# Wallacoloo/libfriendship

Hardware: AMD Instinct MI355X
Metric: Msamples/sec at 4096 partials x 64 voices; achieved HBM GB/s vs roofline (higher is better)
Workload: dtype f32

## Files before the change

libfriendship_amd/csrc/engine.cpp:

```cpp
#include <hip/hip_runtime_api.h>

#include <algorithm>
#include <cfloat>
#include <cmath>
#include <cstdio>
#include <cstdlib>
#include <chrono>
#include <cstring>
#include <map>
#include <sstream>
#include <string>
#include <vector>

#include "../../include/friendship_render_ext.h"
#include "bankplan.hpp"
#include "callplan.hpp"
#include "comm.hpp"
#include "graph.hpp"
#include "jit.hpp"
#include "kernels.hpp"
#include "match.hpp"
#include "stage.hpp"
#include "streamplan.hpp"
#include "streamrows.hpp"
// ... 204 lines not shown
__attribute__((weak)) hipError_t launch_bank_stream_loops(const StreamBanksArgs &, const BankArgs &, const StreamProgArgs &, uint32_t, uint32_t, uint32_t, uint32_t, BankStreamInCtl *,
                                                          BankStreamInDev *, uint32_t, hipStream_t) {
    return hipErrorNotSupported;
}
__attribute__((weak)) hipError_t launch_track_window(const TrackWindowArgs &a, hipStream_t) {
    for (uint32_t r = 0; r < a.n_rows; ++r)
        for (uint64_t i = 0; i < a.back + a.n; ++i)
            a.dst[r][i] = i < a.back ? (a.tail[r] ? a.tail[r][(a.idx - a.back + i) & a.mask] : 0.0f) : (a.call[r] ? a.call[r][i - a.back] : 0.0f);
    return hipSuccess;
}

}

using namespace fr;

struct fr_renderer {
    int device = 0;
    int mode = FR_MODE_AUTO;
    int semantics = FR_SEMANTICS_REFERENCE;
    uint64_t history_frames = 0;
    hipStream_t stream = nullptr;
    Mirror mirror;
    std::vector<InSlot> slots;
    uint64_t n_vecs = 0;
    struct Seg { uint64_t first, last, len; };
    std::vector<Seg> segs;
    uint64_t head = 0;
    Plan plan;
    DevBuf d_out, d_in_table, d_stack_node, d_stack_time, d_stack_val, d_bank_ws, d_tickets;
    PinnedBuf h_in_stage, h_out_stage;
    uint32_t track_from = 0xFFFFFFFFu;
    uint32_t dense_total_rows = 0;
    const float *call_tracks = nullptr;
    uint64_t call_track_stride = 0, call_track_rows = 0;
    DevBuf d_tracks_stage;
    uint64_t track_history = 0, tail_cap = 0;
    DevBuf d_tail, d_track_win;
    uint32_t tail_rows = 0;
    uint64_t tail_end = 0;
    uint64_t tail_launches = 0;
    std::vector<std::pair<uint32_t, DevInput>> track_dev;
    bool tail_on() const { return track_history != 0 && track_from != 0xFFFFFFFFu; }
    DevBuf d_chunk_ws, d_chunk_rows;
    uint32_t d_chunk_rows_n = 0;
    uint32_t stage_block_env = 0;
    bool host_out_mapped = false, host_rows_mapped = true;
    size_t host_small_bytes = 96u << 10;
    bool host_direct = true;
    bool host_stream = true;
    PinnedBuf h_row_flags;
    DevBuf d_row_done;
    uint32_t host_seq = 0;
    std::vector<uint32_t> stream_pending;
    struct FlagOut { uint32_t *host_flags = nullptr; uint32_t *row_done = nullptr; uint32_t value = 0; } flag_out;
    bool can_stream_rows(uint32_t n_slots, uint64_t n_times) const {
        if (!host_stream || sharded() || !plan_current(n_slots) || plan.banks.empty()) return false;
        if (!plan.sp.progs.empty() || plan.sp.uses_rings() || !plan.pull_rows.empty() || !plan.sp.split.empty()) return false;
        size_t voices = 0;
        for (const BankStage &bs : plan.banks) {
            if (!plan_bank_launch(bs, n_times, true).publishes_rows) return false;
            voices += bs.grp.rows.size();
        }
        return voices == n_slots;
    }
    std::vector<std::pair<char *, size_t>> registered;
    bool host_trace = false;
    double trace_us[3] = {0, 0, 0};
    uint64_t trace_n = 0;
    hipEvent_t ev_last = nullptr;
    hipStream_t last_stream = nullptr;
    bool last_pending = false;
    bool last_independent = false;
    bool used_scratch = false;
    bool host_pipelines = false;
    bool overlapped_streams = false;
    bool plan_is_stateless(uint32_t n_slots) const {
        return plan_current(n_slots) && !plan.sp.uses_rings() && plan.sp.progs.empty() && plan.pull_rows.empty() && plan.sp.split.empty() &&
               !tail_on();
    }
    void order_after_previous(hipStream_t st, bool this_independent = false) {
        if (!last_pending) return;
        if (overlapped_streams && !this_independent) {
            HIP_CHECK(hipDeviceSynchronize());
            overlapped_streams = false;
            last_pending = false;
            return;
        }
        if (last_stream == st) return;
        if (last_independent && this_independent) {
            overlapped_streams = true;
            return;
        }
        if (!ev_last) HIP_CHECK(hipEventCreateWithFlags(&ev_last, hipEventDisableTiming));
        if (hipEventRecord(ev_last, last_stream) == hipSuccess) {
            HIP_CHECK(hipStreamWaitEvent(st, ev_last, 0));
        } else {
            (void)hipGetLastError();
            HIP_CHECK(hipDeviceSynchronize());
        }
        last_pending = false;
    }
    void remember_async(hipStream_t st, bool independent) {
        last_independent = independent;
        last_stream = st;
        last_pending = true;
    }
    ShardSpec shard;
    uint32_t shard_flags = 0;
    uint64_t shard_epoch = 0;
    std::unique_ptr<Transport> rccl;
    fr_comm host_comm{};
    bool has_host_comm = false;
    DevBuf d_ws, d_xrecv;
    hipStream_t xstream = nullptr;
    std::vector<hipEvent_t> x_events;
    uint32_t x_max_tiles = 4, x_min_tile = 1024;
    bool x_tiles_explicit = false;
    uint64_t exchange_bytes = 0;
    uint64_t exchange_calls = 0, exchange_tiles = 0;
    PinnedBuf h_xsend, h_xrecv;
    bool sharded() const { return shard.world > 1 && shard.mode != FR_SHARD_NONE; }
// ... 408 lines not shown
            for (uint32_t r = 0; r < n; ++r) if (need[r] && bank_ring[r]) voice_ring[r] = 1;
            while (!work.empty()) {
                const StageProg &pg = sp.progs[work.back()];
                work.pop_back();
                for (uint32_t k = 0; k < pg.n_instr; ++k) {
                    const StageInstr &in = sp.instrs[pg.first_instr + k];
                    if (in.op != S_READ && in.op != S_READ_DYN) continue;
                    if (bank_ring[in.buf]) voice_ring[in.buf] = 1;
                    else if (stored_by[in.buf] >= 0 && !in_set[(size_t)stored_by[in.buf]]) { in_set[(size_t)stored_by[in.buf]] = 1; work.push_back((uint32_t)stored_by[in.buf]); }
                }
            }
            add_voices(voice_ring);
            for (uint32_t r = 0; r < n; ++r) if (voice_ring[r]) now[r].valid_from = 0;
            for (size_t l = 0; l + 1 < sp.fused_level_first.size(); ++l) {
                std::vector<std::pair<uint32_t, uint32_t>> runs;
                for (uint32_t i = f0 + sp.fused_level_first[l]; i < f0 + sp.fused_level_first[l + 1]; ++i) {
                    if (!in_set[i]) continue;
                    add_run(runs, i);
                    for (uint32_t r : sp.prog_rings[i]) now[r].valid_from = 0;
                }
                if (!runs.empty()) rp.levels.push_back(std::move(runs));
            }
        }
        ring_state.repair_from = rp.from;
        ring_table.rings = std::move(now);
        ring_table.shard_epoch = shard_epoch;
        return rp;
    }
    std::vector<hipEvent_t> event_pool;
    std::string last_error;
    std::string jit_error;
    std::string plan_json_cache;

    ~fr_renderer() {
        (void)hipSetDevice(device);
        end_stream();
        for (TimerClass *tc : {&t_bank, &t_pull, &t_stage})
            for (auto &pr : tc->pending) { (void)hipEventDestroy(pr.first); (void)hipEventDestroy(pr.second); }
        for (hipEvent_t e : event_pool) (void)hipEventDestroy(e);
        for (Retired &g : graveyard) (void)hipEventDestroy(g.ev);
        if (ev_last) (void)hipEventDestroy(ev_last);
        if (ev_ring_move) (void)hipEventDestroy(ev_ring_move);
        for (hipEvent_t e : x_events) (void)hipEventDestroy(e);
        if (xstream) (void)hipStreamDestroy(xstream);
        if (!registered.empty()) (void)hipStreamSynchronize(stream);
        for (auto &rg : registered) { if (hipHostUnregister(rg.first) != hipSuccess) (void)hipGetLastError(); }
        if (host_trace && stream_trace_n)
            std::fprintf(stderr, "fr_stream_block over %llu blocks: ring + wait %.1f us, copy out %.1f us\n", (unsigned long long)stream_trace_n,
                         stream_trace_us[0] / stream_trace_n, stream_trace_us[1] / stream_trace_n);
        if (host_trace && trace_n)
            std::fprintf(stderr, "fr_fill_buffer phases over %llu calls (mapped out %d, mapped in %d): issue %.1f us, %s %.1f us, %s %.1f us\n",
                         (unsigned long long)trace_n, (int)host_out_mapped, (int)host_rows_mapped, trace_us[0] / trace_n,
                         host_out_mapped ? "wait" : "D2H issue", trace_us[1] / trace_n, host_out_mapped ? "CPU copy" : "wait", trace_us[2] / trace_n);
        if (stream) (void)hipStreamDestroy(stream);
    }

    uint64_t implicit_len(uint64_t slot) const {
        for (const Seg &s : segs) if (slot >= s.first && slot < s.last) return s.len;
        return 0;
    }

    hipEvent_t get_event() {
        if (!event_pool.empty()) { hipEvent_t e = event_pool.back(); event_pool.pop_back(); return e; }
        hipEvent_t e;
        HIP_CHECK(hipEventCreate(&e));
        return e;
    }
    struct Scope {
        fr_renderer *r; TimerClass *tc; hipStream_t s; hipEvent_t a = nullptr, b = nullptr;
        Scope(fr_renderer *rr, TimerClass *t, hipStream_t st) : r(rr), tc(t), s(st) {
            if (r->timing) { a = r->get_event(); b = r->get_event(); HIP_CHECK(hipEventRecord(a, s)); }
        }
        void done() {
            if (a) { HIP_CHECK(hipEventRecord(b, s)); tc->pending.emplace_back(a, b); a = nullptr; }
        }
    };
    void resolve(TimerClass &tc) {
        for (auto &pr : tc.pending) {
            HIP_CHECK(hipEventSynchronize(pr.second));
            float ms = 0;
            HIP_CHECK(hipEventElapsedTime(&ms, pr.first, pr.second));
            tc.ms += ms;
            tc.launches += 1;
            event_pool.push_back(pr.first);
            event_pool.push_back(pr.second);
        }
        tc.pending.clear();
    }

    bool delay_observed = false;
    uint64_t delay_observed_max = 1u << 20;
    struct Hull {
        float lo = 0.0f, hi = 0.0f;
        uint32_t flags = 0;
        bool known = true;
    };
    std::vector<Hull> hulls;
    uint64_t lookback_growths = 0;
    uint64_t range_launches = 0;
    uint64_t deferred_len = 0;
    PinnedBuf h_range;
    static bool widen(Hull &h, float lo, float hi, uint32_t flags) {
        const bool w = lo < h.lo || hi > h.hi || (flags & ~h.flags) != 0;
        h.lo = std::min(h.lo, lo);
        h.hi = std::max(h.hi, hi);
        h.flags |= flags;
// ... 758 lines not shown
            j.rows = d_chunk_rows.as<uint32_t>();
            j.out_stride = pt.blen;
        }
        if (bs.grp.tracks && pt.trk) {
            j.tracks = pt.trk->p;
            j.track_stride = pt.trk->stride;
            j.track_limit = pt.trk->limit;
        } else if (bs.grp.tracks && call_tracks) {
            if (pt.b0 != c.idx || pt.blen != c.n_times) throw Error(FR_ERR_UNSUPPORTED, "internal: a voice that reads tracks rendered over another window than the call's");
            j.tracks = call_tracks;
            j.track_stride = call_track_stride;
            j.track_limit = (uint32_t)std::min<uint64_t>((uint64_t)track_from + call_track_rows, 0xFFFFFFFFull);
        }
        note_bank_launch(bp, bs, pt.nv, pt.blen, flag_out.host_flags != nullptr);
        Scope sc(this, &t_bank, c.st);
        HIP_CHECK(launch_jit_bank(*bs.jit, j, c.st));
        if (bp.pieces_log2) {
            ChunkCombineArgs cc{};
            cc.ws = d_chunk_ws.as<float>();
            cc.out = a.out;
            cc.rows = a.rows;
            cc.out_stride = a.out_stride;
            cc.n_times = pt.blen;
            cc.n_voices = a.n_voices;
            cc.log2_c = bp.pieces_log2;
            HIP_CHECK(launch_chunk_combine(cc, c.st));
        }
        sc.done();
    }

    void launch_general_bank(const Call &c, BankStage &bs, const BankPart &pt, BankArgs &a) {
        a.groups = bs.d_groups.as<uint32_t>();
        a.group_off = bs.d_group_off.as<uint32_t>();
        a.hist_dst = nullptr;
        note_bank_launch(pt.bp, bs, pt.nv, pt.blen, flag_out.host_flags != nullptr);
        Scope sc(this, &t_bank, c.st);
        HIP_CHECK(launch_gbank(a, c.st));
        sc.done();
    }

    void launch_template_bank(const Call &c, BankStage &bs, const BankPart &pt, BankArgs &a) {
        const BankPlan &bp = pt.bp;
        if (a.hist_dst && !bp.appends_rows) throw Error(FR_ERR_DEVICE, "internal: deferred history append on a short call");
        a.chunk_log2 = bp.chunk_log2;
        a.frames_per_lane = bp.frames_per_lane;
        a.waves_per_group = bp.waves_per_group;
        a.small_call = bp.small_call;
        a.leaf_variant = bank_tune.leaf_variant;
        if (flag_out.host_flags) {
            if (!bp.publishes_rows) throw Error(FR_ERR_DEVICE, "internal: a bank launch cannot publish row flags");
            a.host_flags = flag_out.host_flags;
            a.row_done = flag_out.row_done;
            a.flag_value = flag_out.value;
        }
        if (bp.ws_floats) {
            used_scratch = true;
            d_bank_ws.ensure(bp.ws_floats * sizeof(float));
            a.ws = d_bank_ws.as<float>();
            if (bp.ticket_words) a.tickets = ticket_counters(bp.ticket_words, c.st);
        }
        note_bank_launch(bp, bs, pt.nv, pt.blen, flag_out.host_flags != nullptr);
        Scope sc(this, &t_bank, c.st);
        HIP_CHECK(launch_bank(a, c.st));
        sc.done();
    }

    void launch_bank_window(const Call &c, BankStage &bs, uint64_t b0, uint64_t blen, int64_t tile_off) {
        if (!(bs.grp.tracks && tail_on() && tile_off < 0 && b0 < c.idx && b0 + blen == c.idx + c.n_times)) {
            launch_bank_part(c, bs, b0, blen, tile_off, nullptr);
            return;
        }
        for (uint64_t s0 = b0; s0 < c.idx;) {
            const uint64_t pos = s0 & (tail_cap - 1);
            const uint64_t len = std::min(c.idx - s0, tail_cap - pos);
            TrackSrc ts{nullptr, tail_cap, 0};
            if (tail_rows) {
                ts.p = reinterpret_cast<const float *>(reinterpret_cast<uintptr_t>(d_tail.as<float>() + pos) - (uintptr_t)track_from * tail_cap * sizeof(float));
                ts.limit = (uint32_t)std::min<uint64_t>((uint64_t)track_from + tail_rows, 0xFFFFFFFFull);
            }
            launch_bank_part(c, bs, s0, len, -1, &ts);
            s0 += len;
        }
        launch_bank_part(c, bs, c.idx, c.n_times, -1, nullptr);
    }

    std::vector<DevInput> stage_tab;
    void fill_stage_tab(hipStream_t st) {
        const StagedPlan &sp = plan.sp;
        stage_tab.resize(sp.input_slots.size());
        for (size_t i = 0; i < stage_tab.size(); ++i) stage_tab[i] = dev_input(sp.input_slots[i]);
        if (stage_tab.size() > STAGE_INLINE_INPUTS) {
            d_in_table_stage.ensure(stage_tab.size() * sizeof(DevInput));
            HIP_CHECK(hipMemcpyAsync(d_in_table_stage.p, stage_tab.data(), stage_tab.size() * sizeof(DevInput), hipMemcpyHostToDevice, st));
            HIP_CHECK(hipStreamSynchronize(st));
        }
    }
    struct StageLaunch { const char *form; uint64_t stride; };
    template <class Args>
    void fill_stage_args(Args &a, const Call &c, const StageLaunch &how, uint64_t s0, uint64_t slen, bool carry_only) const {
        a.rings = d_rings.as<float>();
        a.ring_mask = ring_cap ? ring_cap - 1 : 0;
        a.n_inputs = (uint32_t)stage_tab.size();
        a.out = c.dst;
        a.n_times = c.n_times;
        a.idx = c.idx;
        a.w0 = s0;
// ... 630 lines not shown
}
fr_status fr_on_add_edge(fr_renderer *r, const fr_edge *edge) {
    return guarded(r, [&] {
        if (!edge) throw Error(FR_ERR_INVALID_ARG, "null edge");
        r->mirror.add_edge(*edge);
    });
}
fr_status fr_on_del_edge(fr_renderer *r, const fr_edge *edge) {
    return guarded(r, [&] {
        if (!edge) throw Error(FR_ERR_INVALID_ARG, "null edge");
        r->mirror.del_edge(*edge);
    });
}
fr_status fr_on_add_nodes(fr_renderer *r, const uint32_t *handles, const fr_effect *const *effects, size_t n) {
    return guarded(r, [&] {
        if (n && (!handles || !effects)) throw Error(FR_ERR_INVALID_ARG, "null array");
        r->mirror.nodes.reserve(r->mirror.nodes.size() + n);
        for (size_t i = 0; i < n; ++i) r->mirror.add_node(handles[i], effects[i]);
    });
}
fr_status fr_on_add_edges(fr_renderer *r, const fr_edge *edges, size_t n) {
    return guarded(r, [&] {
        if (n && !edges) throw Error(FR_ERR_INVALID_ARG, "null array");
        for (size_t i = 0; i < n; ++i) r->mirror.add_edge(edges[i]);
    });
}

fr_status fr_fill_buffer(fr_renderer *r, float *out, uint32_t n_slots, uint64_t n_times, uint64_t idx,
                         const float *in_data, const uint64_t *in_row_offsets, uint32_t n_in_rows) {
    return guarded(r, [&] {
        check_fill_args(out, n_slots, n_times, in_data, in_row_offsets, n_in_rows);
        HIP_CHECK(hipSetDevice(r->device));
        hipStream_t st = r->stream;
        r->order_after_previous(st);
        r->ensure_plan(n_slots, st);
        const auto snap = r->snapshot_store(idx);
        try {
        r->store_inputs(n_slots, n_times, idx, in_data, in_row_offsets, n_in_rows, false, st);
        size_t bytes = (size_t)n_slots * n_times * sizeof(float);
        uint32_t row_lo, row_hi;
        r->my_rows(n_slots, row_lo, row_hi);
        const bool gather = r->sharded() && (r->shard_flags & FR_SHARD_GATHER);
        using clk = std::chrono::steady_clock;
        const auto t_a = clk::now();
        float *direct = nullptr;
        if (!gather && bytes && r->host_direct)
            for (const auto &rg : r->registered)
                if ((char *)out >= rg.first && (char *)out + bytes <= rg.first + rg.second) {
                    void *dp = nullptr;
                    if (hipHostGetDevicePointer(&dp, out, 0) == hipSuccess) direct = (float *)dp;
                    else (void)hipGetLastError();
                    break;
                }
        if (direct) {
            r->execute(direct, n_slots, n_times, idx, st);
            HIP_CHECK(hipStreamSynchronize(st));
        } else if (bytes >= (256u << 10) && r->can_stream_rows(n_slots, n_times)) {
            r->h_out_stage.ensure(bytes);
            if ((size_t)n_slots * sizeof(uint32_t) > r->h_row_flags.bytes) {
                r->h_row_flags.ensure((size_t)n_slots * 2 * sizeof(uint32_t));
                std::memset(r->h_row_flags.p, 0, r->h_row_flags.bytes);
                r->host_seq = 0;
            }
            r->clean_counters(st);
            if ((size_t)n_slots * sizeof(uint32_t) > r->d_row_done.bytes) {
                r->d_row_done.ensure((size_t)n_slots * 2 * sizeof(uint32_t));
                HIP_CHECK(hipMemsetAsync(r->d_row_done.p, 0, r->d_row_done.bytes, st));
            }
            if (++r->host_seq == 0) {
                std::memset(r->h_row_flags.p, 0, r->h_row_flags.bytes);
                r->host_seq = 1;
            }
            const uint32_t seq = r->host_seq;
            r->flag_out.host_flags = r->h_row_flags.as_dev<uint32_t>();
            r->flag_out.row_done = r->d_row_done.as<uint32_t>();
            r->flag_out.value = seq;
            struct Clear { fr_renderer *r; ~Clear() { r->flag_out = fr_renderer::FlagOut{}; } } clear{r};
            r->execute(r->h_out_stage.as_dev<float>(), n_slots, n_times, idx, st);
            const uint32_t *flags = r->h_row_flags.as<uint32_t>();
            const float *stage = r->h_out_stage.as<float>();
            r->stream_pending.resize(n_slots);
            for (uint32_t i = 0; i < n_slots; ++i) r->stream_pending[i] = i;
            size_t left = n_slots;
            uint64_t idle = 0;
            while (left) {
                bool progress = false;
                for (size_t i = 0; i < left;) {
                    const uint32_t row = r->stream_pending[i];
                    if (__atomic_load_n(flags + row, __ATOMIC_ACQUIRE) == seq) {
                        std::memcpy(out + (size_t)row * n_times, stage + (size_t)row * n_times, n_times * sizeof(float));
                        r->stream_pending[i] = r->stream_pending[--left];
                        progress = true;
                    } else {
                        ++i;
                    }
                }
                if (!progress && (++idle & 0xFFFFu) == 0 && hipStreamQuery(st) != hipErrorNotReady) {
                    HIP_CHECK(hipStreamSynchronize(st));
                    for (size_t i = 0; i < left; ++i)
                        if (__atomic_load_n(flags + r->stream_pending[i], __ATOMIC_ACQUIRE) != seq)
                            throw Error(FR_ERR_DEVICE, "internal: a rendered row was never published to the host");
                }
            }
            HIP_CHECK(hipStreamSynchronize(st));
        } else if ((r->host_out_mapped || bytes <= r->host_small_bytes) && !gather) {
            r->h_out_stage.ensure(bytes);
            r->execute(r->h_out_stage.as_dev<float>(), n_slots, n_times, idx, st);
            const auto t_b = clk::now();
            HIP_CHECK(hipStreamSynchronize(st));
            const auto t_c = clk::now();
            const size_t off = (size_t)row_lo * n_times, cnt = (size_t)(row_hi - row_lo) * n_times;
            if (cnt) std::memcpy(out + off, r->h_out_stage.as<float>() + off, cnt * sizeof(float));
            if (r->host_trace) {
                r->trace_us[0] += std::chrono::duration<double, std::micro>(t_b - t_a).count();
                r->trace_us[1] += std::chrono::duration<double, std::micro>(t_c - t_b).count();
                r->trace_us[2] += std::chrono::duration<double, std::micro>(clk::now() - t_c).count();
                ++r->trace_n;
            }
        } else {
            r->d_out.ensure(bytes);
            r->execute(r->d_out.as<float>(), n_slots, n_times, idx, st);
            if (gather) {
                r->gather_rows(r->d_out.as<float>(), n_slots, n_times, st);
                if (r->shard.rank == 0) { row_lo = 0; row_hi = n_slots; }
            }
            const size_t off = (size_t)row_lo * n_times, cnt = (size_t)(row_hi - row_lo) * n_times;
            const auto t_b = clk::now();
            if (cnt) HIP_CHECK(hipMemcpyAsync(out + off, r->d_out.as<float>() + off, cnt * sizeof(float), hipMemcpyDeviceToHost, st));
            const auto t_c = clk::now();
            HIP_CHECK(hipStreamSynchronize(st));
            if (r->host_trace) {
                r->trace_us[0] += std::chrono::duration<double, std::micro>(t_b - t_a).count();
                r->trace_us[1] += std::chrono::duration<double, std::micro>(t_c - t_b).count();
                r->trace_us[2] += std::chrono::duration<double, std::micro>(clk::now() - t_c).count();
                ++r->trace_n;
            }
        }
        } catch (...) {
            r->rollback_store(snap);
            throw;
        }
        r->last_pending = false;
        r->head = idx + n_times;
    });
}

fr_status fr_fill_buffer_device(fr_renderer *r, float *d_out, uint32_t n_slots, uint64_t n_times, uint64_t idx,
                                const float *d_in_data, const uint64_t *in_row_offsets, uint32_t n_in_rows,
                                void *stream) {
    return guarded(r, [&] {
        check_fill_args(d_out, n_slots, n_times, d_in_data, in_row_offsets, n_in_rows);
        HIP_CHECK(hipSetDevice(r->device));
        hipStream_t st = (hipStream_t)stream;
        bool independent = r->plan_is_stateless(n_slots) && idx == r->head;
        for (uint32_t i = 0; independent && i < n_in_rows; ++i) independent = in_row_offsets[i + 1] - in_row_offsets[i] == n_times;
        r->host_pipelines = independent && r->last_pending && r->last_stream != st;
        struct Reset { fr_renderer *r; ~Reset() { r->host_pipelines = false; } } reset{r};
// ... 442 lines not shown
```

libfriendship_amd/csrc/kernels.hip:

```cpp
#include <hip/hip_runtime.h>

#include <cstdlib>
#include <type_traits>

#include "kernels.hpp"

#pragma clang fp contract(off)

namespace fr {

#ifdef FR_DIAG_STAMPS
__device__ unsigned long long *g_diag = nullptr;
#define FR_DIAG_MARK(slot)                                                                                                 \
    do {                                                                                                                   \
        if (g_diag && (threadIdx.x & 63u) == 0u) {                                                                         \
            unsigned long long v_ = __builtin_amdgcn_s_memrealtime();                                                      \
            if ((slot) == 3) v_ = (unsigned long long)__builtin_amdgcn_s_getreg(0xF804) | ((unsigned long long)(__builtin_amdgcn_s_getreg(0xF814) & 15u) << 32); \
            g_diag[((size_t)blockIdx.x * 16u + (threadIdx.x >> 6)) * 8u + (slot)] = v_;                                    \
            if ((slot) != 3) g_diag[((size_t)blockIdx.x * 16u + (threadIdx.x >> 6)) * 8u + 4u + (slot)] = __builtin_amdgcn_s_memtime(); \
        }                                                                                                                  \
    } while (0)
#else
#define FR_DIAG_MARK(slot) do { } while (0)
#endif
// ... 221 lines not shown
        res[f] = r;
    }
}

__device__ __forceinline__ bool leaves_all_negzero(const float2 *params, uint32_t n, float t, uint32_t tid, uint32_t nthreads) {
    bool ok = true;
    for (uint32_t k = tid; k < n && ok; k += nthreads) {
        float2 p = params[k];
        ok = __float_as_uint(bank_leaf<false, true>(t, p.x, p.y)) == 0x80000000u;
    }
    return ok;
}

template <bool FAST>
__device__ __attribute__((noinline)) bool wave_leaves_all_negzero(const float *params, uint32_t ngroups, float t, unsigned long long lanes) {
    const_f32_ptr p = (const_f32_ptr)params;
    const bool wanted = (lanes >> (threadIdx.x & 63u)) & 1ull;
    uint32_t all_and = 0xFFFFFFFFu, all_or = 0u;
    ParamGroup pa, pb;
    load_group(pa, p, 0);
    auto fold = [&](const ParamGroup &pg) {
#pragma unroll
        for (int j = 0; j < 8; ++j) {
            uint32_t b = __float_as_uint(bank_leaf<FAST, true>(t, pg.w[j], pg.A[j]));
            all_and &= b;
            all_or |= b;
        }
    };
    for (uint32_t g = 0; g < ngroups; g += 2) {
        const bool has_b = g + 1 < ngroups;
        __builtin_amdgcn_s_waitcnt(0xC07F);
        if (has_b) load_group(pb, p, g + 1);
        fold(pa);
        if (has_b) {
            __builtin_amdgcn_s_waitcnt(0xC07F);
            if (g + 2 < ngroups) load_group(pa, p, g + 2);
            fold(pb);
        }
        if (__ballot(wanted && all_and == 0x80000000u && all_or == 0x80000000u) == 0ull) {
            __builtin_amdgcn_s_waitcnt(0xC07F);
            return false;
        }
    }
    return all_and == 0x80000000u && all_or == 0x80000000u;
}

__device__ __forceinline__ float bank_time(const BankArgs &a, uint64_t ti) {
    return (ti >= a.time_skip && ti - a.time_skip < a.time_valid) ? a.time[ti - a.time_skip] : 0.0f;
}
__device__ __forceinline__ uint64_t bank_out_index(const BankArgs &a, uint64_t ti) {
    return a.ring_mask ? ((a.ring_t0 + ti) & a.ring_mask) : ti;
}

template <int F, int MODE, int NW, bool FLAGS = false>
__global__ void __launch_bounds__(64 * NW) bank_kernel(BankArgs a, uint32_t tiles, uint32_t nblocks) {
    uint32_t b = blockIdx.x;
    uint32_t lid = (nblocks % 8u == 0u) ? (b % 8u) * (nblocks / 8u) + b / 8u : b;
    const uint32_t nchunks = 1u << (a.log2_p - a.chunk_log2);
    const uint32_t vc = lid / tiles;
    const uint32_t tile = lid - vc * tiles;
    const uint32_t voice = vc >> (a.log2_p - a.chunk_log2);
    const uint32_t chunk = vc & (nchunks - 1u);
    const uint32_t lane = threadIdx.x & 63u;
    const uint32_t wave = __builtin_amdgcn_readfirstlane(threadIdx.x >> 6);

    FR_DIAG_MARK(0);
    FR_DIAG_MARK(3);
    const uint64_t t0 = (uint64_t)tile * (64u * F);
    float t[F];
    bool nonneg = true;
#pragma unroll
    for (int f = 0; f < F; ++f) {
        uint64_t ti = t0 + (uint32_t)f * 64u + lane;
        t[f] = bank_time(a, ti);
        nonneg = nonneg && (t[f] >= 0.0f) && (t[f] <= 4294967296.0f);
        if (a.hist_dst && vc == 0u && wave == 0u && ti < a.time_valid) a.hist_dst[ti] = t[f];
    }
    const bool fast = a.fast_ok && __all(nonneg);

    const uint32_t Pc = 1u << a.chunk_log2;
    const uint32_t Pw = Pc / NW;
    const float2 *cparams = a.params + ((size_t)voice << a.log2_p) + (size_t)chunk * Pc;
    const float *params = (const float *)(cparams + (size_t)wave * Pw);
    const uint32_t ngroups = Pw >> 3;
    const uint32_t levels = a.chunk_log2 - 3u - (NW == 8 ? 3u : NW == 4 ? 2u : NW == 2 ? 1u : 0u);

    float res[F];
    constexpr bool EXACT = (MODE == 0);
    if (fast) bank_wave_sum<F, true, EXACT>(params, ngroups, levels, t, res);
    else bank_wave_sum<F, false, EXACT>(params, ngroups, levels, t, res);
    FR_DIAG_MARK(1);

    __shared__ float sm[NW][F][64];
    __shared__ unsigned long long zmask[F];
#pragma unroll
    for (int f = 0; f < F; ++f) sm[wave][f][lane] = res[f];
    __syncthreads();
    FR_DIAG_MARK(2);
    const bool direct = nchunks == 1u;
    float *orow = direct ? a.out + (size_t)a.rows[voice] * a.out_stride
                         : a.ws + ((size_t)chunk * a.n_voices + voice) * a.n_times;
    if (wave == 0) {
#pragma unroll
        for (int f = 0; f < F; ++f) {
            uint64_t ti = t0 + (uint32_t)f * 64u + lane;
            float r = sm[0][f][lane];
            if (NW >= 2) r = r + sm[1 % NW][f][lane];
            if (NW >= 4) r = r + (sm[2 % NW][f][lane] + sm[3 % NW][f][lane]);
            if (NW == 8) r = r + ((sm[4 % NW][f][lane] + sm[5 % NW][f][lane]) + (sm[6 % NW][f][lane] + sm[7 % NW][f][lane]));
            bool live = ti < a.n_times;
            if (live) {
                float *dst = &orow[direct ? bank_out_index(a, ti) : ti];
                if (FLAGS) __hip_atomic_store(dst, r, __ATOMIC_RELAXED, __HIP_MEMORY_SCOPE_SYSTEM);
                else __builtin_nontemporal_store(r, dst);
            }
            if (MODE == 1) {
                unsigned long long m = __ballot(live && r == 0.0f);
                if (lane == 0) zmask[f] = m;
            }
        }
    }
    if (MODE == 1) {
        __syncthreads();
#pragma unroll
        for (int f = 0; f < F; ++f) {
            unsigned long long m = zmask[f];
            if (__builtin_popcountll(m) > 4) {
                bool mine = fast ? wave_leaves_all_negzero<true>(params, ngroups, t[f], m)
                                 : wave_leaves_all_negzero<false>(params, ngroups, t[f], m);
                sm[wave][f][lane] = mine ? 1.0f : 0.0f;
                __syncthreads();
                if (wave == 0 && ((m >> lane) & 1ull)) {
                    bool all = true;
#pragma unroll
                    for (int w = 0; w < NW; ++w) all = all && sm[w][f][lane] != 0.0f;
                    uint64_t ti = t0 + (uint32_t)f * 64u + lane;
                    float *dst = &orow[direct ? bank_out_index(a, ti) : ti];
                    if (FLAGS) __hip_atomic_store(dst, all ? -0.0f : 0.0f, __ATOMIC_RELAXED, __HIP_MEMORY_SCOPE_SYSTEM);
                    else *dst = all ? -0.0f : 0.0f;
                }
                __syncthreads();
                continue;
            }
            while (m) {
                uint32_t l = (uint32_t)__builtin_ctzll(m);
                m &= m - 1;
                uint64_t ti = t0 + (uint32_t)f * 64u + l;
                float tz = bank_time(a, ti);
                int all = __syncthreads_and(leaves_all_negzero(cparams, Pc, tz, threadIdx.x, 64u * NW) ? 1 : 0);
                if (threadIdx.x == 0) {
                    float *dst = &orow[direct ? bank_out_index(a, ti) : ti];
                    if (FLAGS) __hip_atomic_store(dst, all ? -0.0f : 0.0f, __ATOMIC_RELAXED, __HIP_MEMORY_SCOPE_SYSTEM);
                    else *dst = all ? -0.0f : 0.0f;
                }
            }
        }
    }
    if (FLAGS && a.host_flags && direct && wave == 0) {
        asm volatile("s_waitcnt vmcnt(0)" ::: "memory");
        if (lane == 0u) {
            const uint32_t old = __hip_atomic_fetch_add(a.row_done + voice, 1u, __ATOMIC_RELAXED, __HIP_MEMORY_SCOPE_AGENT);
            if (old == tiles - 1u) {
                __hip_atomic_store(a.row_done + voice, 0u, __ATOMIC_RELAXED, __HIP_MEMORY_SCOPE_AGENT);
                __hip_atomic_store(a.host_flags + a.rows[voice], a.flag_value, __ATOMIC_RELEASE, __HIP_MEMORY_SCOPE_SYSTEM);
            }
        }
    }
}

template <int F, int MODE>
__global__ void __launch_bounds__(256) bank_multi_kernel(BankArgs a, uint32_t tiles, uint32_t nblocks) {
    uint32_t b = blockIdx.x;
    uint32_t lid = (nblocks % 8u == 0u) ? (b % 8u) * (nblocks / 8u) + b / 8u : b;
    const uint32_t vb = lid / tiles, tile = lid - vb * tiles;
    const uint32_t lane = threadIdx.x & 63u;
    const uint32_t wave = __builtin_amdgcn_readfirstlane(threadIdx.x >> 6);
    const uint64_t t0 = (uint64_t)tile * (64u * F);
    float t[F];
    bool nonneg = true;
#pragma unroll
    for (int f = 0; f < F; ++f) {
        uint64_t ti = t0 + (uint32_t)f * 64u + lane;
        t[f] = bank_time(a, ti);
        nonneg = nonneg && (t[f] >= 0.0f) && (t[f] <= 4294967296.0f);
        if (a.hist_dst && vb == 0u && wave == 0u && ti < a.time_valid) a.hist_dst[ti] = t[f];
    }
    const bool fast = a.fast_ok && __all(nonneg);
    const uint32_t ngroups = 1u << (a.log2_p - 3u), levels = a.log2_p - 3u;
    const uint32_t v0 = (vb * 4u + wave) * a.voices_per_wave;
    constexpr bool EXACT = (MODE == 0);
    for (uint32_t j = 0; j < a.voices_per_wave; ++j) {
        const uint32_t voice = v0 + j;
        if (voice >= a.n_voices) break;
        const float2 *vparams = a.params + ((size_t)voice << a.log2_p);
        float res[F];
        if (fast) bank_wave_sum<F, true, EXACT>((const float *)vparams, ngroups, levels, t, res);
        else bank_wave_sum<F, false, EXACT>((const float *)vparams, ngroups, levels, t, res);
        float *orow = a.out + (size_t)a.rows[voice] * a.out_stride;
#pragma unroll
        for (int f = 0; f < F; ++f) {
            const uint64_t ti = t0 + (uint32_t)f * 64u + lane;
            const bool live = ti < a.n_times;
            if (live) orow[bank_out_index(a, ti)] = res[f];
            if (MODE == 1) {
                unsigned long long zm = __ballot(live && res[f] == 0.0f);
                if (zm == 0ull) continue;
                if (__builtin_popcountll(zm) > 4) {
                    const bool all = fast ? wave_leaves_all_negzero<true>((const float *)vparams, ngroups, t[f], zm)
                                          : wave_leaves_all_negzero<false>((const float *)vparams, ngroups, t[f], zm);
                    if ((zm >> lane) & 1ull) orow[bank_out_index(a, ti)] = all ? -0.0f : 0.0f;
                    continue;
                }
                while (zm) {
                    const uint32_t l = (uint32_t)__builtin_ctzll(zm);
                    zm &= zm - 1;
                    const uint64_t tz_i = t0 + (uint32_t)f * 64u + l;
                    const float tz = bank_time(a, tz_i);
// ... 594 lines not shown
}

__global__ void __launch_bounds__(1024) bank_stream_kernel(BankArgs a, BankStreamCtl *ctl, BankStreamDev *dev, uint32_t idle_ms) {
    __shared__ float sm[STREAM_NW][64];
    __shared__ unsigned long long zshared;
    __shared__ uint32_t s_seq, s_T;
    const uint32_t lane = threadIdx.x & 63u;
    const uint32_t wave = __builtin_amdgcn_readfirstlane(threadIdx.x >> 6);
    const StreamWork w = stream_work(a.params, a.rows, a.log2_p, a.chunk_log2, a.fast_ok, 0u, 0u, blockIdx.x, wave);
    const unsigned long long idle_ticks = (unsigned long long)idle_ms * 100000ull;
    uint32_t seen = 0;
    if (blockIdx.x == 0 && threadIdx.x == 0) __hip_atomic_store(&ctl->alive, 1u, __ATOMIC_RELEASE, __HIP_MEMORY_SCOPE_SYSTEM);
    for (;;) {
        uint32_t T;
        const uint32_t seq = stream_next_block(dev, wave, lane, seen, idle_ticks, s_seq, s_T, T, [&](uint32_t &T0) { return stream_row_wait(ctl, dev, lane, seen, idle_ticks, T0); });
        if (seq == BANK_STREAM_STOP) break;
        seen = seq;
        const bool live = lane < T;
        float t, result;
        const float r = stream_render_chunk(w, dev->row, live, wave, lane, sm, zshared, t);
        if (wave == 0u && stream_hand_over(w, a.ws, a.tickets, a.n_voices, lane, r, result)) {
            if (live) __hip_atomic_store(a.out + (size_t)w.rows[w.bank_voice] * 64u + lane, result, __ATOMIC_RELAXED, __HIP_MEMORY_SCOPE_SYSTEM);
            stream_finish(ctl, dev, a.n_voices, lane, seq);
        }
        __syncthreads();
    }
    if (blockIdx.x == 0 && threadIdx.x == 0) __hip_atomic_store(&ctl->alive, 0u, __ATOMIC_RELEASE, __HIP_MEMORY_SCOPE_SYSTEM);
}

hipError_t launch_bank_stream(const BankArgs &a, BankStreamCtl *ctl_dev, BankStreamDev *dev, uint32_t idle_ms, hipStream_t s) {
    if (!stream_bank_ok(a.log2_p, a.chunk_log2, a.n_voices, a.ws, a.tickets)) return hipErrorInvalidValue;
    if ((1u << a.chunk_log2) / 16u < 8u) return hipErrorInvalidValue;
    if (a.leaf_variant != 1 || !a.out || !a.rows || !ctl_dev || !dev) return hipErrorInvalidValue;
    const uint32_t wgs = a.n_voices << (a.log2_p - a.chunk_log2);
    hipLaunchKernelGGL(bank_stream_kernel, dim3(wgs), dim3(1024), 0, s, a, ctl_dev, dev, idle_ms ? idle_ms : BANK_STREAM_IDLE_MS);
    return hipGetLastError();
}

uint64_t bank_blocks(const BankArgs &a) {
    uint64_t f = a.frames_per_lane;
    return ((a.n_times + 64 * f - 1) / (64 * f)) * a.n_voices << (a.log2_p - a.chunk_log2);
}

template <int F>
static hipError_t launch_bank_f(const BankArgs &a, hipStream_t s) {
    uint64_t nblocks64 = bank_blocks(a);
    if (nblocks64 == 0) return hipSuccess;
    if (nblocks64 > 0x7FFFFFFFull) return hipErrorInvalidValue;
    uint32_t tiles = (uint32_t)((a.n_times + 64 * F - 1) / (64 * F)), nblocks = (uint32_t)nblocks64;
    const bool w8 = a.waves_per_group == 8;
    if (a.leaf_variant == 0) {
        if (w8) hipLaunchKernelGGL((bank_kernel<F, 0, 8>), dim3(nblocks), dim3(512), 0, s, a, tiles, nblocks);
        else hipLaunchKernelGGL((bank_kernel<F, 0, 4>), dim3(nblocks), dim3(256), 0, s, a, tiles, nblocks);
    } else if (a.leaf_variant == 1 && a.host_flags && a.chunk_log2 == a.log2_p) {
        if (w8) hipLaunchKernelGGL((bank_kernel<F, 1, 8, true>), dim3(nblocks), dim3(512), 0, s, a, tiles, nblocks);
        else hipLaunchKernelGGL((bank_kernel<F, 1, 4, true>), dim3(nblocks), dim3(256), 0, s, a, tiles, nblocks);
    } else if (a.leaf_variant == 1) {
        if (w8) hipLaunchKernelGGL((bank_kernel<F, 1, 8>), dim3(nblocks), dim3(512), 0, s, a, tiles, nblocks);
        else if (a.waves_per_group == 2 && a.chunk_log2 <= 12) hipLaunchKernelGGL((bank_kernel<F, 1, 2>), dim3(nblocks), dim3(128), 0, s, a, tiles, nblocks);
        else if (a.waves_per_group == 1 && a.chunk_log2 <= 11) hipLaunchKernelGGL((bank_kernel<F, 1, 1>), dim3(nblocks), dim3(64), 0, s, a, tiles, nblocks);
        else hipLaunchKernelGGL((bank_kernel<F, 1, 4>), dim3(nblocks), dim3(256), 0, s, a, tiles, nblocks);
    } else {
        hipLaunchKernelGGL((bank_kernel<F, 2, 4>), dim3(nblocks), dim3(256), 0, s, a, tiles, nblocks);
    }
    hipError_t e = hipGetLastError();
    if (e != hipSuccess || a.chunk_log2 == a.log2_p) return e;
    uint64_t total = (uint64_t)a.n_voices * a.n_times;
    hipLaunchKernelGGL(bank_combine_kernel, dim3((uint32_t)((total + 255) / 256)), dim3(256), 0, s, a);
    return hipGetLastError();
}

hipError_t launch_bank(const BankArgs &a, hipStream_t s) {
    if (a.small_call == 2) {
        if (a.chunk_log2 < 7 || a.chunk_log2 > 13 || a.chunk_log2 > a.log2_p || a.log2_p - a.chunk_log2 > 8) return hipErrorInvalidValue;
        if (a.chunk_log2 != a.log2_p && (!a.ws || !a.tickets)) return hipErrorInvalidValue;
        if ((8u << a.chunk_log2) / (8u * a.waves_per_group) < 8u) return hipErrorInvalidValue;
        switch (a.waves_per_group) {
        case 4: return launch_bank_short<4>(a, s);
        case 8: return launch_bank_short<8>(a, s);
        case 16: return launch_bank_short<16>(a, s);
        default: return hipErrorInvalidValue;
        }
    }
    if (a.small_call) {
        if (a.log2_p < 8 || a.log2_p > 24 || a.n_times > SMALL_MAX_FRAMES || a.chunk_log2 != 8) return hipErrorInvalidValue;
        if (a.log2_p != 8 && !a.ws) return hipErrorInvalidValue;
        if (a.n_times == 0 || a.n_voices == 0) return hipSuccess;
        if (a.n_voices > 65535u) return hipErrorInvalidValue;
        hipLaunchKernelGGL(bank_small_kernel, dim3(1u << (a.log2_p - 8u), a.n_voices), dim3(256), 0, s, a);
        hipError_t e = hipGetLastError();
        if (e != hipSuccess || a.log2_p == 8) return e;
        uint64_t total = (uint64_t)a.n_voices * a.n_times;
        hipLaunchKernelGGL(bank_combine_kernel, dim3((uint32_t)((total + 255) / 256)), dim3(256), 0, s, a);
        return hipGetLastError();
    }
    if (a.voices_per_wave) {
        if (a.log2_p < 3 || a.log2_p > 8 || a.chunk_log2 != a.log2_p || a.voices_per_wave > 64) return hipErrorInvalidValue;
        if (a.n_times == 0 || a.n_voices == 0) return hipSuccess;
        const uint32_t F = a.frames_per_lane;
        if (F != 1 && F != 2) return hipErrorInvalidValue;
        const uint64_t tiles = (a.n_times + 64 * F - 1) / (64 * F);
        const uint64_t vgroups = ((uint64_t)a.n_voices + 4ull * a.voices_per_wave - 1) / (4ull * a.voices_per_wave);
        const uint64_t nb = tiles * vgroups;
        if (nb > 0x7FFFFFFFull) return hipErrorInvalidValue;
        const int mode = a.leaf_variant > 2 ? 1 : (int)a.leaf_variant;
        if (F == 1) {
            if (mode == 0) hipLaunchKernelGGL((bank_multi_kernel<1, 0>), dim3((uint32_t)nb), dim3(256), 0, s, a, (uint32_t)tiles, (uint32_t)nb);
            else if (mode == 1) hipLaunchKernelGGL((bank_multi_kernel<1, 1>), dim3((uint32_t)nb), dim3(256), 0, s, a, (uint32_t)tiles, (uint32_t)nb);
            else hipLaunchKernelGGL((bank_multi_kernel<1, 2>), dim3((uint32_t)nb), dim3(256), 0, s, a, (uint32_t)tiles, (uint32_t)nb);
        } else {
            if (mode == 0) hipLaunchKernelGGL((bank_multi_kernel<2, 0>), dim3((uint32_t)nb), dim3(256), 0, s, a, (uint32_t)tiles, (uint32_t)nb);
            else if (mode == 1) hipLaunchKernelGGL((bank_multi_kernel<2, 1>), dim3((uint32_t)nb), dim3(256), 0, s, a, (uint32_t)tiles, (uint32_t)nb);
            else hipLaunchKernelGGL((bank_multi_kernel<2, 2>), dim3((uint32_t)nb), dim3(256), 0, s, a, (uint32_t)tiles, (uint32_t)nb);
        }
        return hipGetLastError();
    }
    if (a.waves_per_group != 4 && a.waves_per_group != 8 && a.waves_per_group != 2 && a.waves_per_group != 1) return hipErrorInvalidValue;
    if (a.waves_per_group < 4 && (a.leaf_variant != 1 || a.host_flags)) return hipErrorInvalidValue;
    const uint32_t cmin = a.waves_per_group == 8 ? 6 : a.waves_per_group == 4 ? 5 : a.waves_per_group == 2 ? 4 : 3;
    const uint32_t cmax = a.waves_per_group == 8 ? 14 : a.waves_per_group == 4 ? 13 : a.waves_per_group == 2 ? 12 : 11;
    if (a.log2_p < cmin || a.log2_p > 24 || a.chunk_log2 < cmin || a.chunk_log2 > cmax || a.chunk_log2 > a.log2_p)
        return hipErrorInvalidValue;
    if (a.chunk_log2 != a.log2_p && !a.ws) return hipErrorInvalidValue;
    switch (a.frames_per_lane) {
    case 1: return launch_bank_f<1>(a, s);
    case 2: return launch_bank_f<2>(a, s);
    case 4: return launch_bank_f<4>(a, s);
    default: return hipErrorInvalidValue;
    }
}

constexpr uint32_t GB_MAX_DEPTH = 16;

template <bool FAST>
__device__ __forceinline__ float gbank_group(const ParamGroup &pg, uint32_t j, float t) {
    float l0 = bank_leaf<FAST, false>(t, pg.w[0], pg.A[0]);
    float v = l0;
    if (j >= 1u) {
        float l1 = bank_leaf<FAST, false>(t, pg.w[1], pg.A[1]);
        v = l0 + l1;
        if (j >= 2u) {
            float l2 = bank_leaf<FAST, false>(t, pg.w[2], pg.A[2]);
            float l3 = bank_leaf<FAST, false>(t, pg.w[3], pg.A[3]);
            v = v + (l2 + l3);
            if (j >= 3u) {
                float l4 = bank_leaf<FAST, false>(t, pg.w[4], pg.A[4]);
                float l5 = bank_leaf<FAST, false>(t, pg.w[5], pg.A[5]);
                float l6 = bank_leaf<FAST, false>(t, pg.w[6], pg.A[6]);
                float l7 = bank_leaf<FAST, false>(t, pg.w[7], pg.A[7]);
                v = v + ((l4 + l5) + (l6 + l7));
            }
        }
    }
    return v;
}

template <bool FAST>
__device__ __forceinline__ float gbank_tile(const float *params, const uint32_t *gmeta, uint32_t nitems, float t, uint32_t wave, uint32_t lane,
                                            float *stack , float (*sm)[64]) {
    uint32_t sp = 0;
    const_f32_ptr p = (const_f32_ptr)params;
    typedef uint32_t __attribute__((address_space(4))) const *const_u32_ptr;
    const_u32_ptr gm = (const_u32_ptr)gmeta;
    auto finish = [&](float v, uint32_t meta) {
        for (uint32_t m = meta >> 4; m != 0u; --m) {
            --sp;
            v = stack[sp * 64u] + v;
        }
        stack[sp * 64u] = v;
        ++sp;
    };
// ... 890 lines not shown
```

libfriendship_amd/csrc/kernels.hpp:

```cpp
#pragma once

#include <hip/hip_runtime_api.h>

#include <cstdint>

namespace fr {

struct DevInput {
    const float *data;
    uint64_t base;
    uint64_t len;
};

struct DevNode {
    uint32_t op, a, b, depth;
};

struct PullArgs {
    const DevNode *nodes;
    const uint32_t *outputs;
    const DevInput *inputs;
    uint32_t n_inputs;
    float *out;
    uint32_t n_slots;
    uint64_t n_times;
    uint64_t idx;
    uint64_t first;
    uint64_t count;
    uint32_t sparkle;
    uint32_t *st_node;
    uint64_t *st_time;
    float *st_val;
};
hipError_t launch_pull(const PullArgs &a, hipStream_t s);

struct BankArgs {
    const float2 *params;
    const float *time;
    uint64_t time_skip;
    uint64_t time_valid;
    float *out;
    const uint32_t *rows;
    uint64_t out_stride;
    uint64_t ring_mask;
    uint64_t ring_t0;
    uint32_t n_voices;
    uint32_t log2_p;
    uint64_t n_times;
    uint32_t fast_ok;
    uint32_t chunk_log2;
    uint32_t frames_per_lane;
    uint32_t waves_per_group;
    uint32_t small_call;
    uint32_t voices_per_wave;
    uint32_t leaf_variant;
    float *hist_dst;
    float *ws;
    uint32_t *row_done;
    uint32_t *host_flags;
    uint32_t flag_value;
    uint32_t *tickets;
    const uint32_t *groups;
    const uint32_t *group_off;
};
constexpr uint32_t BANK_TICKET_STRIDE = 32;

struct BankStreamCtl {
    unsigned long long row[64];
    uint32_t done;
    uint32_t alive;
    uint32_t pad1[14];
};
struct BankStreamDev {
    uint32_t seq;
    uint32_t n_times;
    uint32_t voices_done;
    uint32_t pad[13];
    float row[64];
};
constexpr uint32_t BANK_STREAM_STOP = 0xFFFFFFFFu;
constexpr uint32_t BANK_STREAM_WGS = 256;
constexpr uint32_t BANK_STREAM_IDLE_MS = 2000;
hipError_t launch_bank_stream(const BankArgs &a, BankStreamCtl *ctl_dev, BankStreamDev *dev, uint32_t idle_ms, hipStream_t s);
uint64_t bank_blocks(const BankArgs &a);
hipError_t launch_bank(const BankArgs &a, hipStream_t s);
hipError_t launch_gbank(const BankArgs &a, hipStream_t s);

enum StageOp : uint8_t {
    S_CONST = 0,
    S_INPUT = 1,
    S_READ = 2,
    S_READ_INPUT = 3,
    S_STEP = 4,
    S_SUM2 = 5, S_MUL = 6, S_DIV = 7, S_MOD = 8, S_MIN = 9,
    S_STORE = 10,
    S_READ_DYN = 11,
    S_READ_INPUT_DYN = 12,
    S_STEP_DYN = 13,
};
struct StageInstr {
    uint8_t op, dst, a, b;
    uint32_t imm;
    uint32_t buf;
    uint32_t d_lo;
};
struct StageProg {
    uint32_t first_instr, n_instr;
    uint32_t result_reg;
    uint32_t dst_ring;
    int32_t out_row;
    uint32_t n_loads;
    uint32_t pad[2];
};
constexpr int STAGE_REGS = 48;
constexpr uint32_t STAGE_INLINE_INPUTS = 8;
constexpr uint32_t STAGE_MAX_HOISTED = 24;
// ... 166 lines not shown
```

Before: 40.64.

## Stage streamed rows in device memory and push completed rows to host in-kernel

When host output is directly mapped and rows can be streamed, the bank kernel now writes tiles to a device-side staging buffer with agent-scope stores. The last tile to finish a row copies the whole row to the host-mapped destination using vectorized system-coherent dwordx4 stores, then publishes the row flag. This replaces many scattered system-scope scalar atomic stores across PCIe with bulk vector writes, and drops the CPU memcpy from the pinned stage when writing directly. It also adds host-side phase tracing. The cost is an extra device read-back pass per row and a serialized push by one workgroup per row.

Result: no change. 40.48 (-0.4%).

```diff
diff --git a/libfriendship_amd/csrc/engine.cpp b/libfriendship_amd/csrc/engine.cpp
--- a/libfriendship_amd/csrc/engine.cpp
+++ b/libfriendship_amd/csrc/engine.cpp
@@ -280,7 +280,7 @@
     DevBuf d_row_done;
     uint32_t host_seq = 0;
     std::vector<uint32_t> stream_pending;
-    struct FlagOut { uint32_t *host_flags = nullptr; uint32_t *row_done = nullptr; uint32_t value = 0; } flag_out;
+    struct FlagOut { uint32_t *host_flags = nullptr; uint32_t *row_done = nullptr; uint32_t value = 0; float *row_stage = nullptr; } flag_out;
     bool can_stream_rows(uint32_t n_slots, uint64_t n_times) const {
         if (!host_stream || sharded() || !plan_current(n_slots) || plan.banks.empty()) return false;
         if (!plan.sp.progs.empty() || plan.sp.uses_rings() || !plan.pull_rows.empty() || !plan.sp.split.empty()) return false;
@@ -295,6 +295,8 @@
     bool host_trace = false;
     double trace_us[3] = {0, 0, 0};
     uint64_t trace_n = 0;
+    double rows_trace_us[4] = {0, 0, 0, 0};
+    uint64_t rows_trace_n = 0;
     hipEvent_t ev_last = nullptr;
     hipStream_t last_stream = nullptr;
     bool last_pending = false;
@@ -809,6 +811,10 @@
             std::fprintf(stderr, "fr_fill_buffer phases over %llu calls (mapped out %d, mapped in %d): issue %.1f us, %s %.1f us, %s %.1f us\n",
                          (unsigned long long)trace_n, (int)host_out_mapped, (int)host_rows_mapped, trace_us[0] / trace_n,
                          host_out_mapped ? "wait" : "D2H issue", trace_us[1] / trace_n, host_out_mapped ? "CPU copy" : "wait", trace_us[2] / trace_n);
+        if (host_trace && rows_trace_n)
+            std::fprintf(stderr, "fr_fill_buffer streamed-row phases over %llu calls: issue %.1f us, launch -> last flag %.1f us (row copies %.1f us of it), trailing synchronize %.1f us\n",
+                         (unsigned long long)rows_trace_n, rows_trace_us[0] / rows_trace_n, rows_trace_us[1] / rows_trace_n, rows_trace_us[2] / rows_trace_n,
+                         rows_trace_us[3] / rows_trace_n);
         if (stream) (void)hipStreamDestroy(stream);
     }
 
@@ -1673,6 +1679,7 @@
             a.host_flags = flag_out.host_flags;
             a.row_done = flag_out.row_done;
             a.flag_value = flag_out.value;
+            a.row_stage = flag_out.row_stage;
         }
         if (bp.ws_floats) {
             used_scratch = true;
@@ -2409,11 +2416,13 @@
                     else (void)hipGetLastError();
                     break;
                 }
-        if (direct) {
+        const bool stream_rows = !gather && bytes >= (256u << 10) && r->can_stream_rows(n_slots, n_times);
+        if (direct && !stream_rows) {
             r->execute(direct, n_slots, n_times, idx, st);
             HIP_CHECK(hipStreamSynchronize(st));
-        } else if (bytes >= (256u << 10) && r->can_stream_rows(n_slots, n_times)) {
-            r->h_out_stage.ensure(bytes);
+        } else if (stream_rows) {
+            if (!direct) r->h_out_stage.ensure(bytes);
+            float *const dst = direct ? direct : r->h_out_stage.as_dev<float>();
             if ((size_t)n_slots * sizeof(uint32_t) > r->h_row_flags.bytes) {
                 r->h_row_flags.ensure((size_t)n_slots * 2 * sizeof(uint32_t));
                 std::memset(r->h_row_flags.p, 0, r->h_row_flags.bytes);
@@ -2429,23 +2438,29 @@
                 r->host_seq = 1;
             }
             const uint32_t seq = r->host_seq;
+            r->d_out.ensure(bytes + 16);
             r->flag_out.host_flags = r->h_row_flags.as_dev<uint32_t>();
             r->flag_out.row_done = r->d_row_done.as<uint32_t>();
             r->flag_out.value = seq;
+            r->flag_out.row_stage = r->d_out.as<float>() + (((uintptr_t)dst >> 2) & 3u);
             struct Clear { fr_renderer *r; ~Clear() { r->flag_out = fr_renderer::FlagOut{}; } } clear{r};
-            r->execute(r->h_out_stage.as_dev<float>(), n_slots, n_times, idx, st);
+            r->execute(dst, n_slots, n_times, idx, st);
             const uint32_t *flags = r->h_row_flags.as<uint32_t>();
             const float *stage = r->h_out_stage.as<float>();
             r->stream_pending.resize(n_slots);
             for (uint32_t i = 0; i < n_slots; ++i) r->stream_pending[i] = i;
-            size_t left = n_slots;
+            size_t left = direct ? 0 : n_slots;
             uint64_t idle = 0;
+            const auto t_b = clk::now();
+            double copy_us = 0;
             while (left) {
                 bool progress = false;
                 for (size_t i = 0; i < left;) {
                     const uint32_t row = r->stream_pending[i];
                     if (__atomic_load_n(flags + row, __ATOMIC_ACQUIRE) == seq) {
+                        const auto t_r = r->host_trace ? clk::now() : t_b;
                         std::memcpy(out + (size_t)row * n_times, stage + (size_t)row * n_times, n_times * sizeof(float));
+                        if (r->host_trace) copy_us += std::chrono::duration<double, std::micro>(clk::now() - t_r).count();
                         r->stream_pending[i] = r->stream_pending[--left];
                         progress = true;
                     } else {
@@ -2459,7 +2474,15 @@
                             throw Error(FR_ERR_DEVICE, "internal: a rendered row was never published to the host");
                 }
             }
+            const auto t_c = clk::now();
             HIP_CHECK(hipStreamSynchronize(st));
+            if (r->host_trace && !direct) {
+                r->rows_trace_us[0] += std::chrono::duration<double, std::micro>(t_b - t_a).count();
+                r->rows_trace_us[1] += std::chrono::duration<double, std::micro>(t_c - t_b).count();
+                r->rows_trace_us[2] += copy_us;
+                r->rows_trace_us[3] += std::chrono::duration<double, std::micro>(clk::now() - t_c).count();
+                ++r->rows_trace_n;
+            }
         } else if ((r->host_out_mapped || bytes <= r->host_small_bytes) && !gather) {
             r->h_out_stage.ensure(bytes);
             r->execute(r->h_out_stage.as_dev<float>(), n_slots, n_times, idx, st);
diff --git a/libfriendship_amd/csrc/kernels.hip b/libfriendship_amd/csrc/kernels.hip
--- a/libfriendship_amd/csrc/kernels.hip
+++ b/libfriendship_amd/csrc/kernels.hip
@@ -297,6 +297,37 @@
     return a.ring_mask ? ((a.ring_t0 + ti) & a.ring_mask) : ti;
 }
 
+__device__ __forceinline__ void bank_flag_store(float *dst, float v, bool staged) {
+    if (staged) __hip_atomic_store(dst, v, __ATOMIC_RELAXED, __HIP_MEMORY_SCOPE_AGENT);
+    else __hip_atomic_store(dst, v, __ATOMIC_RELAXED, __HIP_MEMORY_SCOPE_SYSTEM);
+}
+
+typedef float bank_f32x4 __attribute__((ext_vector_type(4)));
+template <uint32_t NT>
+__device__ __forceinline__ void bank_push_row(const float *src, float *dst, uint64_t n) {
+    uint64_t head = (4u - (uint32_t)((uintptr_t)dst >> 2)) & 3u;
+    if (head > n) head = n;
+    const uint64_t quads = (n - head) >> 2, tail0 = head + quads * 4u;
+    if (threadIdx.x < head) bank_flag_store(dst + threadIdx.x, src[threadIdx.x], false);
+    if (threadIdx.x < n - tail0) bank_flag_store(dst + tail0 + threadIdx.x, src[tail0 + threadIdx.x], false);
+    const bank_f32x4 *src4 = (const bank_f32x4 *)(src + head);
+    bank_f32x4 *dst4 = (bank_f32x4 *)(dst + head);
+    for (uint64_t q0 = threadIdx.x; q0 < quads; q0 += 8ull * NT) {
+        bank_f32x4 v[8];
+#pragma unroll
+        for (uint32_t u = 0; u < 8u; ++u) {
+            const uint64_t q = q0 + (uint64_t)u * NT;
+            v[u] = src4[q < quads ? q : quads - 1u];
+        }
+#pragma unroll
+        for (uint32_t u = 0; u < 8u; ++u) {
+            const uint64_t q = q0 + (uint64_t)u * NT;
+            if (q < quads) asm volatile("global_store_dwordx4 %0, %1, off sc0 sc1\n\ts_nop 1" ::"v"(dst4 + q), "v"(v[u]) : "memory");
+        }
+        if (q0 + 8ull * NT < quads) asm volatile("s_waitcnt vmcnt(0)" ::: "memory");
+    }
+}
+
 template <int F, int MODE, int NW, bool FLAGS = false>
 __global__ void __launch_bounds__(64 * NW) bank_kernel(BankArgs a, uint32_t tiles, uint32_t nblocks) {
     uint32_t b = blockIdx.x;
@@ -343,7 +374,8 @@
     __syncthreads();
     FR_DIAG_MARK(2);
     const bool direct = nchunks == 1u;
-    float *orow = direct ? a.out + (size_t)a.rows[voice] * a.out_stride
+    const bool staged = FLAGS && direct && a.row_stage != nullptr && tiles > 1u;
+    float *orow = direct ? (staged ? a.row_stage : a.out) + (size_t)a.rows[voice] * a.out_stride
                          : a.ws + ((size_t)chunk * a.n_voices + voice) * a.n_times;
     if (wave == 0) {
 #pragma unroll
@@ -356,7 +388,7 @@
             bool live = ti < a.n_times;
             if (live) {
                 float *dst = &orow[direct ? bank_out_index(a, ti) : ti];
-                if (FLAGS) __hip_atomic_store(dst, r, __ATOMIC_RELAXED, __HIP_MEMORY_SCOPE_SYSTEM);
+                if (FLAGS) bank_flag_store(dst, r, staged);
                 else __builtin_nontemporal_store(r, dst);
             }
             if (MODE == 1) {
@@ -381,7 +413,7 @@
                     for (int w = 0; w < NW; ++w) all = all && sm[w][f][lane] != 0.0f;
                     uint64_t ti = t0 + (uint32_t)f * 64u + lane;
                     float *dst = &orow[direct ? bank_out_index(a, ti) : ti];
-                    if (FLAGS) __hip_atomic_store(dst, all ? -0.0f : 0.0f, __ATOMIC_RELAXED, __HIP_MEMORY_SCOPE_SYSTEM);
+                    if (FLAGS) bank_flag_store(dst, all ? -0.0f : 0.0f, staged);
                     else *dst = all ? -0.0f : 0.0f;
                 }
                 __syncthreads();
@@ -395,19 +427,45 @@
                 int all = __syncthreads_and(leaves_all_negzero(cparams, Pc, tz, threadIdx.x, 64u * NW) ? 1 : 0);
                 if (threadIdx.x == 0) {
                     float *dst = &orow[direct ? bank_out_index(a, ti) : ti];
-                    if (FLAGS) __hip_atomic_store(dst, all ? -0.0f : 0.0f, __ATOMIC_RELAXED, __HIP_MEMORY_SCOPE_SYSTEM);
+                    if (FLAGS) bank_flag_store(dst, all ? -0.0f : 0.0f, staged);
                     else *dst = all ? -0.0f : 0.0f;
                 }
             }
         }
     }
-    if (FLAGS && a.host_flags && direct && wave == 0) {
-        asm volatile("s_waitcnt vmcnt(0)" ::: "memory");
-        if (lane == 0u) {
-            const uint32_t old = __hip_atomic_fetch_add(a.row_done + voice, 1u, __ATOMIC_RELAXED, __HIP_MEMORY_SCOPE_AGENT);
-            if (old == tiles - 1u) {
-                __hip_atomic_store(a.row_done + voice, 0u, __ATOMIC_RELAXED, __HIP_MEMORY_SCOPE_AGENT);
-                __hip_atomic_store(a.host_flags + a.rows[voice], a.flag_value, __ATOMIC_RELEASE, __HIP_MEMORY_SCOPE_SYSTEM);
+    if constexpr (FLAGS) {
+        if (a.row_done && direct && !staged) {
+            if (wave == 0) {
+                asm volatile("s_waitcnt vmcnt(0)" ::: "memory");
+                if (lane == 0u) {
+                    const uint32_t old = __hip_atomic_fetch_add(a.row_done + voice, 1u, __ATOMIC_RELAXED, __HIP_MEMORY_SCOPE_AGENT);
+                    if (old == tiles - 1u) {
+                        __hip_atomic_store(a.row_done + voice, 0u, __ATOMIC_RELAXED, __HIP_MEMORY_SCOPE_AGENT);
+                        if (a.host_flags) __hip_atomic_store(a.host_flags + a.rows[voice], a.flag_value, __ATOMIC_RELEASE, __HIP_MEMORY_SCOPE_SYSTEM);
+                    }
+                }
+            }
+        } else if (a.row_done && staged) {
+            __shared__ uint32_t row_last;
+            if (wave == 0) {
+                asm volatile("s_waitcnt vmcnt(0)" ::: "memory");
+                if (lane == 0u) {
+                    const uint32_t old = __hip_atomic_fetch_add(a.row_done + voice, 1u, __ATOMIC_RELAXED, __HIP_MEMORY_SCOPE_AGENT);
+                    row_last = old == tiles - 1u ? 1u : 0u;
+                    if (old == tiles - 1u) __builtin_amdgcn_fence(__ATOMIC_ACQUIRE, "agent");
+                }
+                asm volatile("s_waitcnt vmcnt(0)" ::: "memory");
+            }
+            __syncthreads();
+            if (row_last) {
+                const size_t off = (size_t)a.rows[voice] * a.out_stride;
+                bank_push_row<64u * NW>(a.row_stage + off, a.out + off, a.n_times);
+                asm volatile("s_waitcnt vmcnt(0)" ::: "memory");
+                __syncthreads();
+                if (threadIdx.x == 0u) {
+                    __hip_atomic_store(a.row_done + voice, 0u, __ATOMIC_RELAXED, __HIP_MEMORY_SCOPE_AGENT);
+                    if (a.host_flags) __hip_atomic_store(a.host_flags + a.rows[voice], a.flag_value, __ATOMIC_RELEASE, __HIP_MEMORY_SCOPE_SYSTEM);
+                }
             }
         }
     }
@@ -1108,7 +1166,9 @@
     if (a.leaf_variant == 0) {
         if (w8) hipLaunchKernelGGL((bank_kernel<F, 0, 8>), dim3(nblocks), dim3(512), 0, s, a, tiles, nblocks);
         else hipLaunchKernelGGL((bank_kernel<F, 0, 4>), dim3(nblocks), dim3(256), 0, s, a, tiles, nblocks);
-    } else if (a.leaf_variant == 1 && a.host_flags && a.chunk_log2 == a.log2_p) {
+    } else if (a.leaf_variant == 1 && (a.host_flags || a.row_stage) && a.chunk_log2 == a.log2_p) {
+        if (!a.row_done) return hipErrorInvalidValue;
+        if (a.row_stage && (a.ring_mask || (((uintptr_t)a.row_stage ^ (uintptr_t)a.out) & 15u))) return hipErrorInvalidValue;
         if (w8) hipLaunchKernelGGL((bank_kernel<F, 1, 8, true>), dim3(nblocks), dim3(512), 0, s, a, tiles, nblocks);
         else hipLaunchKernelGGL((bank_kernel<F, 1, 4, true>), dim3(nblocks), dim3(256), 0, s, a, tiles, nblocks);
     } else if (a.leaf_variant == 1) {
@@ -1172,7 +1232,7 @@
         return hipGetLastError();
     }
     if (a.waves_per_group != 4 && a.waves_per_group != 8 && a.waves_per_group != 2 && a.waves_per_group != 1) return hipErrorInvalidValue;
-    if (a.waves_per_group < 4 && (a.leaf_variant != 1 || a.host_flags)) return hipErrorInvalidValue;
+    if (a.waves_per_group < 4 && (a.leaf_variant != 1 || a.host_flags || a.row_stage)) return hipErrorInvalidValue;
     const uint32_t cmin = a.waves_per_group == 8 ? 6 : a.waves_per_group == 4 ? 5 : a.waves_per_group == 2 ? 4 : 3;
     const uint32_t cmax = a.waves_per_group == 8 ? 14 : a.waves_per_group == 4 ? 13 : a.waves_per_group == 2 ? 12 : 11;
     if (a.log2_p < cmin || a.log2_p > 24 || a.chunk_log2 < cmin || a.chunk_log2 > cmax || a.chunk_log2 > a.log2_p)
diff --git a/libfriendship_amd/csrc/kernels.hpp b/libfriendship_amd/csrc/kernels.hpp
--- a/libfriendship_amd/csrc/kernels.hpp
+++ b/libfriendship_amd/csrc/kernels.hpp
@@ -62,6 +62,7 @@
     uint32_t *tickets;
     const uint32_t *groups;
     const uint32_t *group_off;
+    float *row_stage;
 };
 constexpr uint32_t BANK_TICKET_STRIDE = 32;
 
```
